# microsoft/Sora

Hardware: AMD Instinct MI355X
Metric: IQ Msamples/s through 802.11a 54 Mbps RX PHY (higher is better)
Workload: dtype int16 IQ / u8 path metrics

## Files before the change

### sora_amd/csrc/dev_vit16.h

```cpp
#pragma once
#include <hip/hip_runtime.h>
#include "kernels.h"
#include "dev_viterbi.h"

namespace sora {
namespace {

template <int WIN, int LOOK> struct Geom16 {
    static constexpr int kMaxWalk = (WIN + LOOK + 7) / 8 + 2;
    static constexpr int P = kMaxWalk;
    static constexpr int kPathBytes = 40;
};

template <int WIN, int LOOK> struct Lds16 {
    uint16_t ring[Geom16<WIN, LOOK>::P][4][64];
    union {
        uint32_t udump[4][64];
        uint16_t ops[4][24][2];
        uint16_t ops2[2][4][24][2];
    };
    uint32_t path[8][Geom16<WIN, LOOK>::kPathBytes / 4];
};

constexpr unsigned kW[4] = { 0u, 21u, 42u, 63u };

__device__ __forceinline__ unsigned v_of_lane(unsigned l)
{
    const unsigned b0 = l & 1u, b1 = (l >> 1) & 1u, b2 = (l >> 2) & 1u, b3 = (l >> 3) & 1u;
    const unsigned c3 = b2, c1 = b3, c0 = b0 ^ c3, c2 = b1 ^ c3;
    return c0 | (c1 << 1) | (c2 << 2) | (c3 << 3);
}
__device__ __forceinline__ unsigned lane_of_v(unsigned v)
{
    const unsigned c0 = v & 1u, c1 = (v >> 1) & 1u, c2 = (v >> 2) & 1u, c3 = (v >> 3) & 1u;
    return c0 ^ (c2 << 1) ^ (c1 << 3) ^ (c3 ? 7u : 0u);
}
__device__ __forceinline__ unsigned rev6u(unsigned x) { return __brev(x) >> 26; }

template <int CTRL> __device__ __forceinline__ unsigned dppx(unsigned v) { return (unsigned)__builtin_amdgcn_update_dpp(0, (int)v, CTRL, 0xF, 0xF, true); }

__device__ __forceinline__ unsigned partner(unsigned v, int ph)
{
    switch (ph) {
    case 0: return dppx<0x140>(v);
    case 1: return dppx<0x1B>(v);
    case 2: return dppx<0x141>(v);
    case 3: return dppx<0x4E>(v);
    case 4: return dppx<0x128>(v);
    default: return dppx<0xB1>(v);
    }
}

struct Vit16 {
    unsigned U[4];
    unsigned MX[24];
    unsigned MY[6];
    unsigned sadr[3][4];
};

template <int WHICH, int P>
__device__ __forceinline__ void acs16(Vit16& V, int t24, unsigned a, unsigned b, unsigned pos512[3])
{
    const int ph = t24 % 6, k = t24 % 8;
    const unsigned Kp = (WHICH == 0 ? 14u : 7u) * kFld + (kOne << k);
    unsigned bm;
    if (WHICH == 0)      bm = (a ^ V.MX[t24]) + (b ^ V.MY[ph]);
    else if (WHICH == 1) bm = a ^ V.MX[t24];
    else                 bm = b ^ V.MX[t24];
    const unsigned bo = Kp - bm;
    const int rx = ph == 0 ? 2 : ph == 1 ? 1 : 0;
    unsigned N[4];
#pragma unroll
    for (int i = 0; i < 4; i++) {
        const unsigned X = V.U[i], Y = partner(V.U[i ^ rx], ph);
        const bool wb = (kW[i] >> (5 - ph)) & 1u;
        N[i] = wb ? pk_min16(X + bo, Y + bm) : pk_min16(X + bm, Y + bo);
    }
#pragma unroll
    for (int i = 0; i < 4; i++) V.U[i] = N[i];
    if (k == 7) {
        const int jb = t24 / 8;
#pragma unroll
        for (int i = 0; i < 4; i++) {
            const unsigned w = bank_word(V.U[i]);
            const unsigned addr = V.sadr[jb][i] + pos512[jb];
            asm volatile("ds_write_b16 %0, %1" : : "v"(addr), "v"(w) : "memory");
            V.U[i] &= 0xFE00FE00u;
        }
    }
}

__device__ __forceinline__ unsigned row_min_u32(unsigned v)
{
    v = min(v, dppx<0xB1>(v)); v = min(v, dppx<0x4E>(v)); v = min(v, dppx<0x141>(v)); v = min(v, dppx<0x128>(v));
    return v;
}
__device__ __forceinline__ unsigned row_pkmin(unsigned v)
{
    v = pk_min16(v, dppx<0xB1>(v)); v = pk_min16(v, dppx<0x4E>(v)); v = pk_min16(v, dppx<0x141>(v)); v = pk_min16(v, dppx<0x128>(v));
    return v;
}
__device__ __forceinline__ unsigned wave_min_u32(unsigned v) { return (unsigned)__builtin_amdgcn_readfirstlane((int)dpp_min_u32_wave(v)); }
__device__ __forceinline__ unsigned wave_max_u32(unsigned v) { return ~wave_min_u32(~v); }

template <int CR, int WIN, int LOOK, int BITS>
struct Forward16 {
    static constexpr int P = Geom16<WIN, LOOK>::P, GB = Puncture<CR>::GB, GS = Puncture<CR>::GS, CW = Puncture<CR>::CW;
    static constexpr int NV = Puncture<CR>::NV;
    struct Chunk { uint32_t v[CW]; };
    struct Raw { SoftRaw r[NV]; };

    Vit16 V;
    unsigned row, half;
    uint32_t my_j;
    SoftCursor<BITS, CW> cur[NV];
    uint32_t my_base;
    const uint8_t* soft;
    uint16_t* my_ops;
    const uint4* row_ops;
    uint32_t pos;
    unsigned pos512[3];
    uint32_t tr, nsteps;
    uint32_t next_thr;
    bool all_done;

    __device__ __forceinline__ void init(Lds16<WIN, LOOK>& S, const uint8_t* __restrict__ soft_, uint32_t my_soft_off, uint32_t my_first, uint32_t my_last, unsigned start,
                                         uint32_t nsteps_)
    {
        const unsigned lane = threadIdx.x & 63, l16 = lane & 15;
        row = lane >> 4; half = lane & 1u;
        const unsigned v0 = v_of_lane(l16);
        nsteps = nsteps_;
#pragma unroll
        for (int i = 0; i < 4; i++) V.U[i] = (v0 ^ kW[i]) == 0 ? 0u : start;
        const unsigned ring_base = (unsigned)(uintptr_t)&S.ring[0][0][0];
#pragma unroll
        for (int jb = 0; jb < 3; jb++)
#pragma unroll
            for (int i = 0; i < 4; i++) V.sadr[jb][i] = ring_base + ((row * 64u + rev6u(rol6(v0 ^ kW[i], jb == 0 ? 2 : jb == 1 ? 4 : 0))) << 1);
#pragma unroll
        for (int t = 0; t < 24; t++) {
            const int ph = t % 6, k = t % 8;
            const unsigned n = rol6(v0, ph + 1);
            const bool vb = (v0 >> (5 - ph)) & 1u;
            const unsigned ma = (__popc(n & 0155) & 1) ? 7u * kFld : 0u, mb = (__popc(n & 0117) & 1) ? 7u * kFld : 0u;
            const unsigned mx = Puncture<CR>::which_of(ph) == 2 ? mb : ma;
            V.MX[t] = vb ? ((mx ^ (7u * kFld)) | (kOne << k)) : mx;
            if (t < 6) V.MY[t] = vb ? (mb ^ (7u * kFld)) : mb;
        }
        tr = 0; pos = 0;
        my_j = l16 >> 1;
#pragma unroll
        for (int v = 0; v < NV; v++) cur[v].init(my_soft_off, my_first + my_j + 8u * v, my_last);
        my_base = my_soft_off + my_first + my_j;
        soft = soft_;
        my_ops = &S.ops[row][my_j][half];
        row_ops = reinterpret_cast<const uint4*>(&S.ops[row][0][0]);
        set_row_pos();
        clear_ops(S);
    }
    __device__ __forceinline__ bool going() const { return tr < nsteps && !all_done; }

    __device__ __forceinline__ void normalize()
    {
        const unsigned m = row_pkmin(pk_min16(pk_min16(V.U[0], V.U[1]), pk_min16(V.U[2], V.U[3])));
#pragma unroll
        for (int i = 0; i < 4; i++) V.U[i] -= m;
    }
    static __device__ __forceinline__ uint32_t pos_of(uint32_t p, int jb) { const uint32_t q = p + 512u * (uint32_t)jb; return min(q, q - 512u * (uint32_t)P); }
    __device__ __forceinline__ void set_row_pos()
    {
        pos512[0] = pos; pos512[1] = pos_of(pos, 1); pos512[2] = pos_of(pos512[1], 1);
    }
    __device__ __forceinline__ void end_row() { pos = pos_of(pos512[2], 1); set_row_pos(); }
    __device__ __forceinline__ Raw fetch(uint32_t c) const
    {
        Raw R;
#pragma unroll
        for (int v = 0; v < NV; v++) R.r[v] = cur[v].fetch(soft, c);
        return R;
    }
    __device__ __forceinline__ void put(const Raw& R, uint16_t* mine) const
    {
#pragma unroll
        for (int v = 0; v < NV; v++) soft_put(mine + 16 * v, cur[v], R.r[v]);
    }
    __device__ __forceinline__ void clear_ops(Lds16<WIN, LOOK>& S) const
    {
        if constexpr (BITS == kSoftScaled) {
            static_assert(sizeof(S.ops2) == 3 * 64 * 4, "three dwords per lane");
            uint32_t* z = reinterpret_cast<uint32_t*>(&S.ops2[0][0][0][0]) + (threadIdx.x & 63);
            z[0] = 0u; z[64] = 0u; z[128] = 0u;
            lds_fence();
        }
    }
    __device__ __forceinline__ uint32_t fast_base(uint32_t c0) const { return my_base + c0 * (uint32_t)CW; }
    template <int DC> __device__ __forceinline__ Raw fetch_at(uint32_t p) const
    {
        static_assert(BITS == kSoftScaled, "one byte per value");
        Raw R;
#pragma unroll
        for (int v = 0; v < NV; v++) { R.r[v].sh = 0; R.r[v].w = soft[(size_t)p + (size_t)(DC * CW + 8 * v)]; }
        return R;
    }
    static __device__ __forceinline__ Chunk get(const uint4* table)
    {
        Chunk K;
#pragma unroll
        for (int i = 0; i < (CW + 3) / 4; i++) {
            const uint4 x = table[i];
            K.v[4 * i] = x.x; K.v[4 * i + 1] = x.y;
            if (4 * i + 2 < CW) { K.v[4 * i + 2] = x.z; K.v[4 * i + 3] = x.w; }
        }
        return K;
    }
    __device__ __forceinline__ Chunk unpack(const Raw& R) const
    {
        put(R, my_ops);
        lds_fence();
        const Chunk K = get(row_ops);
        lds_fence();
        return K;
    }
    __device__ __forceinline__ void group(const Chunk& K, int h, int i0)
    {
        const int k0 = i0 / GS * GB, t24 = 12 * h + i0;
        acs16<0, P>(V, t24, K.v[k0], K.v[k0 + 1], pos512);
        if (CR != 0) acs16<1, P>(V, t24 + 1, K.v[k0 + 2], 0, pos512);
        if (CR == 2) acs16<2, P>(V, t24 + 2, 0, K.v[k0 + 3], pos512);
        if ((t24 + GS) % 8 == 0) normalize();
    }
    __device__ __forceinline__ void fast_chunk(const Chunk& K, int h)
    {
#pragma unroll
        for (int g = 0; g < 12 / GS; g++) group(K, h, g * GS);
        tr += 12;
    }
    template <typename CHECK> __device__ __forceinline__ void slow_chunk(const Chunk& K, int h, CHECK& check)
    {
#pragma unroll
        for (int g = 0; g < 12 / GS; g++) {
            if (going()) {
                group(K, h, g * GS);
                tr += GS;
                check(12 * h + g * GS + GS - 1);
            }
        }
    }
    template <typename CHECK> __device__ __forceinline__ void chunk(const Chunk& K, int h, CHECK& check)
    {
        if (tr + 12 <= nsteps && next_thr > tr + 12) fast_chunk(K, h); else slow_chunk(K, h, check);
    }
};

template <int WIN, int LOOK, bool LANE_OB = false>
__device__ __noinline__ void trace16(unsigned lds_off, unsigned U0, unsigned U1, unsigned U2, unsigned U3, uint32_t tr_, uint32_t ob_, uint32_t pj_, uint32_t k_,
                                     uint32_t my_cnt, uint8_t* my_out)
{
    using G = Geom16<WIN, LOOK>;
    constexpr int P = G::P, K = G::kMaxWalk;
    constexpr int NR = K - 1, NF = NR / 4, NW = K / 4 + 1;
    static_assert(NR % 4 == 0 || NR % 4 == 2, "the walk's words are packed in pairs");
    static_assert(NW * 4 <= G::kPathBytes && NW >= WIN / 32 + 1, "the stream's registers hold a window and fit Lds16::path");
    typedef __attribute__((address_space(3))) Lds16<WIN, LOOK> lds_t;
    typedef __attribute__((address_space(3))) const uint16_t lds_u16;
    lds_t& S = *(lds_t*)(uintptr_t)lds_off;
    auto uni = [](uint32_t v) { return (uint32_t)__builtin_amdgcn_readfirstlane((int)v); };
    const uint32_t tr = uni(tr_), ob = LANE_OB ? ob_ : uni(ob_), pj = uni(pj_), k = uni(k_);
    const unsigned lane = threadIdx.x & 63, row = lane >> 4, l16 = lane & 15, half = lane & 1u;
    const unsigned v0 = v_of_lane(l16);
    const unsigned U[4] = { U0, U1, U2, U3 };
    const uint32_t j = (tr - 1) >> 3, nn = tr - 8u * j, m_lo = ob >> 3;
    const unsigned rowbase = (unsigned)(uintptr_t)&S.ring[0][row][0], sh = 8u * half;
    auto ring_j = [&](unsigned idx) -> unsigned { return *(lds_u16*)(uintptr_t)(rowbase + pj + (idx << 1)); };
#pragma unroll
    for (int i = 0; i < 4; i++) S.udump[i][lane] = U[i];
    lds_fence();
    unsigned key[2] = { 0xFFFFFFFFu, 0xFFFFFFFFu };
#pragma unroll
    for (int i = 0; i < 4; i++) {
        const unsigned st = rol6(v0 ^ kW[i], tr);
        unsigned lastA, lastB;
        if (k == 7) { const unsigned w = ring_j(rev6u(st)); lastA = (w >> 7) & 1u; lastB = (w >> 15) & 1u; }
        else { lastA = (U[i] >> k) & 1u; lastB = (U[i] >> (17 + k)) & 1u; }
        const unsigned mA = ((U[i] & 0xFFFFu) >> 9 << 1) | lastA, mB = (U[i] >> 25 << 1) | lastB;
        key[0] = min(key[0], (mA << 8) | (st << 2)); key[1] = min(key[1], (mB << 8) | (st << 2));
    }
    const unsigned kA = row_min_u32(key[0]), kB = row_min_u32(key[1]);
    const unsigned st = ((half ? kB : kA) >> 2) & 0x3Fu;
    const unsigned s0 = rol6(st, 6u - tr % 6u);
    const unsigned b4 = (s0 >> 4) & 1u, b5 = (s0 >> 5) & 1u;
    const unsigned ri = b4 | (b5 << 1);
    const unsigned sl = lane_of_v((s0 ^ (b4 ? 21u : 0u) ^ (b5 ? 42u : 0u)) & 15u);
    const unsigned Ust = S.udump[ri][row * 16u + sl];
    unsigned H;
    if (nn == 8) H = (ring_j(rev6u(st)) >> sh) & 0xFFu;
    else H = ((Ust >> (17u * half)) & 0xFFu) & ((1u << nn) - 1u);
    unsigned q = rev6u(((st >> nn) | rev6u(H & 0x3Fu)) & 0x3Fu);
    unsigned pr[NR / 2];
    uint32_t p = pj;
#pragma unroll
    for (int i = 1; i < K; i++) {
        uint32_t d;
        p = __builtin_sub_overflow(p, 512u, &d) ? 512u * (uint32_t)(P - 1) : d;
        unsigned base = rowbase + p;
        asm volatile("" : "+v"(base));
        const unsigned raw = *(lds_u16*)(uintptr_t)(base + (q << 1));
        q = __builtin_amdgcn_ubfe(raw, sh, 6u);
        const int s = K - 1 - i;
        if (s & 1) pr[s >> 1] = raw << 16; else pr[s >> 1] |= raw;
    }
    unsigned R[NW];
    const unsigned sel = 0x06040200u + 0x01010101u * half;
#pragma unroll
    for (int w = 0; w < NF; w++) R[w] = __builtin_amdgcn_perm(pr[2 * w + 1], pr[2 * w], sel);
    if (NR % 4 == 0) R[NF] = H;
    else R[NF] = __builtin_amdgcn_perm(H, pr[2 * NF], 0x0C040200u + 0x00000101u * half);
    const uint32_t sfirst = (uint32_t)(K - 1) - (j - m_lo);
    bool fast = !LANE_OB;
    if (!LANE_OB) {
        const bool whole = my_cnt == (uint32_t)WIN && sfirst == 1u && (((uintptr_t)my_out + m_lo) & 3u) == 0;
        fast = __ballot(!(whole || my_cnt == 0)) == 0;
    }
    if (fast) {
        if (my_cnt != 0 && l16 < 2) {
            uint32_t* o = reinterpret_cast<uint32_t*>(my_out + m_lo);
#pragma unroll
            for (int dw = 0; dw < WIN / 32; dw++) o[dw] = __builtin_amdgcn_alignbit(R[dw + 1], R[dw], 14);
        }
    } else {
        __attribute__((address_space(3))) uint32_t* pw = S.path[row * 2u + half];
        if (l16 < 2) {
#pragma unroll
            for (int w = 0; w < NW; w++) pw[w] = R[w];
        }
        lds_fence();
        __attribute__((address_space(3))) const uint8_t* pth = (__attribute__((address_space(3))) const uint8_t*)pw;
        const uint32_t nbytes = my_cnt >> 3;
        for (uint32_t z = l16 >> 1; z < nbytes; z += 8) {
            const uint32_t sb = sfirst + z;
            my_out[m_lo + z] = (uint8_t)(((unsigned)pth[sb] >> 6) | (((unsigned)pth[sb + 1] & 0x3Fu) << 2));
        }
    }
    lds_fence();
}

}
}
```

### sora_amd/csrc/k_vit16.hip

```cpp
#include <hip/hip_runtime.h>

#include "dev_vit16.h"

namespace sora {

namespace {

template <int CR, int WIN, int LOOK, int BITS>
__device__ __forceinline__ void forward16(Lds16<WIN, LOOK>& S, const uint8_t* __restrict__ soft, uint32_t my_soft_off, uint32_t my_nsoft,
                                          uint32_t nstepsA, uint32_t nstepsB, uint32_t my_tr_end, bool my_valid, uint8_t* my_out)
{
    using F16 = Forward16<CR, WIN, LOOK, BITS>;
    using Chunk = typename F16::Chunk;
    using Raw = typename F16::Raw;
    constexpr int GS = F16::GS;
    F16 F;
    F.init(S, soft, my_soft_off, 0, max(my_nsoft, 1u) - 1u, 0x18u * kFld, wave_max_u32(max(nstepsA, nstepsB)));

    uint32_t ob = 0;
    bool my_done = !my_valid;

    auto trace = [&](uint32_t my_cnt, int t24_last) {
        trace16<WIN, LOOK>((unsigned)(uintptr_t)&S, F.V.U[0], F.V.U[1], F.V.U[2], F.V.U[3], F.tr, ob, F16::pos_of(F.pos, t24_last / 8), (uint32_t)(t24_last % 8), my_cnt, my_out);
    };
    auto next_event = [&]() -> uint32_t {
        const uint32_t mine = my_done ? kNever : my_tr_end;
        return min(ob + (uint32_t)(WIN + LOOK + 6), wave_min_u32(mine));
    };
    F.next_thr = next_event();
    F.all_done = wave_min_u32(my_done ? 1u : 0u) != 0u;
    auto check = [&](int t24_last) {
        if (F.tr >= F.next_thr) {
            const bool partial = F.tr >= ob + (uint32_t)(WIN + LOOK + 6);
            uint32_t cnt = 0;
            if (!my_done) {
                if (F.tr >= my_tr_end) { cnt = my_tr_end - ob - 6; my_done = true; }
                else if (partial) cnt = WIN;
            }
            if (wave_max_u32(cnt) != 0u) { trace(cnt, t24_last); F.clear_ops(S); }
            if (partial) ob += WIN;
            F.next_thr = next_event();
            F.all_done = wave_min_u32(my_done ? 1u : 0u) != 0u;
        }
    };

    uint16_t* my_ops2[2] = { &S.ops2[0][F.row][F.my_j][F.half], &S.ops2[1][F.row][F.my_j][F.half] };
    const uint4* row_ops2[2] = { reinterpret_cast<const uint4*>(&S.ops2[0][F.row][0][0]), reinterpret_cast<const uint4*>(&S.ops2[1][F.row][0][0]) };
    auto stage = [&](const Raw& R, int t) { F.put(R, my_ops2[t]); };
    auto collect = [&](int t) -> Chunk { lds_fence(); return F16::get(row_ops2[t]); };
    auto fast_chunk_mid = [&](const Chunk& K, int h, Chunk& Knext, int tnext) {
#pragma unroll
        for (int g = 0; g < 12 / GS; g++) {
            if (g == (12 / GS) / 2) Knext = collect(tnext);
            F.group(K, h, g * GS);
        }
        F.tr += 12;
    };

    uint32_t c = 0;
    Raw b0 = F.fetch(0), b1 = F.fetch(1), b2, b3;
    while (F.going()) {
        const uint32_t lim = min(F.nsteps, F.next_thr - 1);
        uint32_t rows = lim > F.tr ? (lim - F.tr) / 24 : 0;
        if (rows >= 2) {
            Chunk Ka, Kb;
            b2 = F.fetch(c + 2);
            stage(b0, 0); Ka = collect(0); lds_fence();
            if constexpr (BITS == kSoftScaled) {
                uint32_t p = F.fast_base(c);
                for (; rows >= 2; rows -= 2) {
                    b3 = F.template fetch_at<3>(p); stage(b1, 1); fast_chunk_mid(Ka, 0, Kb, 1);
                    b0 = F.template fetch_at<4>(p); stage(b2, 0); fast_chunk_mid(Kb, 1, Ka, 0);
                    F.end_row();
                    b1 = F.template fetch_at<5>(p); stage(b3, 1); fast_chunk_mid(Ka, 0, Kb, 1);
                    b2 = F.template fetch_at<6>(p); stage(b0, 0); fast_chunk_mid(Kb, 1, Ka, 0);
                    F.end_row();
                    c += 4; p += 4u * (uint32_t)F16::CW;
                }
            } else {
                for (; rows >= 2; rows -= 2) {
                    b3 = F.fetch(c + 3); stage(b1, 1); fast_chunk_mid(Ka, 0, Kb, 1);
                    b0 = F.fetch(c + 4); stage(b2, 0); fast_chunk_mid(Kb, 1, Ka, 0);
                    F.end_row();
                    b1 = F.fetch(c + 5); stage(b3, 1); fast_chunk_mid(Ka, 0, Kb, 1);
                    b2 = F.fetch(c + 6); stage(b0, 0); fast_chunk_mid(Kb, 1, Ka, 0);
                    F.end_row();
                    c += 4;
                }
            }
            lds_fence();
        }
        if (!(F.tr < F.nsteps)) break;
        b2 = F.fetch(c + 2);
        if (rows) F.fast_chunk(F.unpack(b0), 0); else F.chunk(F.unpack(b0), 0, check);
        if (!F.going()) break;
        b3 = F.fetch(c + 3);
        if (rows) F.fast_chunk(F.unpack(b1), 1); else F.chunk(F.unpack(b1), 1, check);
        F.end_row();
        b0 = b2; b1 = b3;
        c += 2;
    }
}

template <int WIN, int LOOK, int BITS>
__device__ __forceinline__ void viterbi16_body(const VitJob* __restrict__ jobs, const uint32_t* __restrict__ njobs3, uint32_t njobs_single, uint32_t stride,
                                               const uint8_t* __restrict__ soft, uint8_t* __restrict__ out)
{
    __shared__ Lds16<WIN, LOOK> S;
    uint32_t n[3] = { njobs_single, 0, 0 };
    if (njobs3) { n[0] = njobs3[0]; n[1] = njobs3[1]; n[2] = njobs3[2]; }
    uint32_t w = uni(blockIdx.x), list = 0;
    while (list < 3 && w >= (n[list] + 7) / 8) { w -= (n[list] + 7) / 8; list++; }
    if (list >= 3) return;
    const uint32_t njobs = uni(n[list]);
    jobs += (size_t)list * stride;
    const unsigned lane = threadIdx.x & 63, row = lane >> 4, half = lane & 1u;
    const uint32_t fa = 8u * w + 2u * row, fb = fa + 1u;
    const bool hasA = fa < njobs, hasB = fb < njobs;
    const VitJob& GA = jobs[hasA ? fa : 8u * w];
    const VitJob& GBj = jobs[hasB ? fb : (hasA ? fa : 8u * w)];
    const uint32_t code_rate = uni(jobs[8u * w].code_rate);
    const uint32_t gsd = code_rate == 0 ? 2u : code_rate == 2 ? 4u : 3u, gss = code_rate == 0 ? 1u : code_rate == 2 ? 3u : 2u;
    const uint32_t nstepsA = hasA ? GA.nsoft / gsd * gss : 0u, nstepsB = hasB ? GBj.nsoft / gsd * gss : 0u;
    const VitJob& Mine = half ? GBj : GA;
    const bool my_valid = half ? hasB : hasA;
    const uint32_t my_tr_end = Mine.length * 8u + 16u + 6u;
    uint8_t* my_out = out + Mine.out_off;
    if (code_rate == 0)      forward16<0, WIN, LOOK, BITS>(S, soft, Mine.soft_off, Mine.nsoft, nstepsA, nstepsB, my_tr_end, my_valid, my_out);
    else if (code_rate == 1) forward16<1, WIN, LOOK, BITS>(S, soft, Mine.soft_off, Mine.nsoft, nstepsA, nstepsB, my_tr_end, my_valid, my_out);
    else                     forward16<2, WIN, LOOK, BITS>(S, soft, Mine.soft_off, Mine.nsoft, nstepsA, nstepsB, my_tr_end, my_valid, my_out);
}

}

__global__ void __launch_bounds__(64) k_viterbi16(const VitJob* __restrict__ jobs, const uint32_t* __restrict__ njobs3, uint32_t njobs_single, uint32_t stride,
        const uint8_t* __restrict__ soft, uint8_t* __restrict__ out)
{ viterbi16_body<256, 24, kSoftScaled>(jobs, njobs3, njobs_single, stride, soft, out); }
__global__ void __launch_bounds__(64) k_viterbi16_p3(const VitJob* __restrict__ jobs, const uint32_t* __restrict__ njobs3, uint32_t njobs_single, uint32_t stride,
        const uint8_t* __restrict__ soft, uint8_t* __restrict__ out)
{ viterbi16_body<256, 24, 3>(jobs, njobs3, njobs_single, stride, soft, out); }
__global__ void __launch_bounds__(64) k_viterbi16_11n(const VitJob* __restrict__ jobs, const uint32_t* __restrict__ njobs3, uint32_t njobs_single,
        uint32_t stride, const uint8_t* __restrict__ soft, uint8_t* __restrict__ out)
{ viterbi16_body<192, 36, 8>(jobs, njobs3, njobs_single, stride, soft, out); }

}
```

Baseline: 55870.

## Overlap Viterbi traceback walk with forward ACS steps in 16-bit decoder

When a full window is ready and conditions allow, the traceback is started but its per-step LDS walk is interleaved with the next two rows of forward ACS groups via a hook, instead of running as a separate serial trace. Survivor bank writes that would overwrite ring entries still needed by the walk are held in registers and flushed once the walk finishes. This aims to hide traceback latency behind forward compute, at the cost of more registers, more code paths and a fallback when alignment or window conditions fail.

```diff
diff --git a/sora_amd/csrc/dev_vit16.h b/sora_amd/csrc/dev_vit16.h
--- a/sora_amd/csrc/dev_vit16.h
+++ b/sora_amd/csrc/dev_vit16.h
@@ -87,6 +87,46 @@
             asm volatile("ds_write_b16 %0, %1" : : "v"(addr), "v"(w) : "memory");
             V.U[i] &= 0xFE00FE00u;
         }
+    }
+}
+
+struct BankStore16 {
+    __device__ __forceinline__ void operator()(const Vit16& V, const unsigned pos512[3], int jb, const unsigned w[4]) const
+    {
+#pragma unroll
+        for (int i = 0; i < 4; i++) {
+            const unsigned addr = V.sadr[jb][i] + pos512[jb];
+            asm volatile("ds_write_b16 %0, %1" : : "v"(addr), "v"(w[i]) : "memory");
+        }
+    }
+};
+
+template <int WHICH, int P, typename BANK>
+__device__ __forceinline__ void acs16(Vit16& V, int t24, unsigned a, unsigned b, unsigned pos512[3], BANK&& bank)
+{
+    const int ph = t24 % 6, k = t24 % 8;
+    const unsigned Kp = (WHICH == 0 ? 14u : 7u) * kFld + (kOne << k);
+    unsigned bm;
+    if (WHICH == 0)      bm = (a ^ V.MX[t24]) + (b ^ V.MY[ph]);
+    else if (WHICH == 1) bm = a ^ V.MX[t24];
+    else                 bm = b ^ V.MX[t24];
+    const unsigned bo = Kp - bm;
+    const int rx = ph == 0 ? 2 : ph == 1 ? 1 : 0;
+    unsigned N[4];
+#pragma unroll
+    for (int i = 0; i < 4; i++) {
+        const unsigned X = V.U[i], Y = partner(V.U[i ^ rx], ph);
+        const bool wb = (kW[i] >> (5 - ph)) & 1u;
+        N[i] = wb ? pk_min16(X + bo, Y + bm) : pk_min16(X + bm, Y + bo);
+    }
+#pragma unroll
+    for (int i = 0; i < 4; i++) V.U[i] = N[i];
+    if (k == 7) {
+        const int jb = t24 / 8;
+        unsigned w[4];
+#pragma unroll
+        for (int i = 0; i < 4; i++) { w[i] = bank_word(V.U[i]); V.U[i] &= 0xFE00FE00u; }
+        bank(V, pos512, jb, w);
     }
 }
 
@@ -250,6 +290,37 @@
     template <typename CHECK> __device__ __forceinline__ void chunk(const Chunk& K, int h, CHECK& check)
     {
         if (tr + 12 <= nsteps && next_thr > tr + 12) fast_chunk(K, h); else slow_chunk(K, h, check);
+    }
+    struct NoHook { __device__ __forceinline__ void operator()(int) const {} };
+    template <typename HOOK, typename BANK> __device__ __forceinline__ void group(const Chunk& K, int h, int i0, HOOK&& hook, BANK&& bank)
+    {
+        const int k0 = i0 / GS * GB, t24 = 12 * h + i0;
+        hook(t24);
+        acs16<0, P>(V, t24, K.v[k0], K.v[k0 + 1], pos512, bank);
+        if (CR != 0) { hook(t24 + 1); acs16<1, P>(V, t24 + 1, K.v[k0 + 2], 0, pos512, bank); }
+        if (CR == 2) { hook(t24 + 2); acs16<2, P>(V, t24 + 2, 0, K.v[k0 + 3], pos512, bank); }
+        if ((t24 + GS) % 8 == 0) normalize();
+    }
+    template <typename BANK> __device__ __forceinline__ void fast_chunk(const Chunk& K, int h, BANK&& bank)
+    {
+#pragma unroll
+        for (int g = 0; g < 12 / GS; g++) group(K, h, g * GS, NoHook{}, bank);
+        tr += 12;
+    }
+    template <typename CHECK, typename BANK> __device__ __forceinline__ void slow_chunk(const Chunk& K, int h, CHECK& check, BANK&& bank)
+    {
+#pragma unroll
+        for (int g = 0; g < 12 / GS; g++) {
+            if (going()) {
+                group(K, h, g * GS, NoHook{}, bank);
+                tr += GS;
+                check(12 * h + g * GS + GS - 1);
+            }
+        }
+    }
+    template <typename CHECK, typename BANK> __device__ __forceinline__ void chunk(const Chunk& K, int h, CHECK& check, BANK&& bank)
+    {
+        if (tr + 12 <= nsteps && next_thr > tr + 12) fast_chunk(K, h, bank); else slow_chunk(K, h, check, bank);
     }
 };
 
@@ -345,5 +416,106 @@
     lds_fence();
 }
 
-}
-}
+template <int WIN, int LOOK>
+__device__ __forceinline__ void trace16_start(unsigned lds_off, const unsigned U[4], uint32_t tr, uint32_t pj, uint32_t k, unsigned& H_, unsigned& q_)
+{
+    typedef __attribute__((address_space(3))) Lds16<WIN, LOOK> lds_t;
+    typedef __attribute__((address_space(3))) const uint16_t lds_u16;
+    lds_t& S = *(lds_t*)(uintptr_t)lds_off;
+    const unsigned lane = threadIdx.x & 63, row = lane >> 4, l16 = lane & 15, half = lane & 1u;
+    const unsigned v0 = v_of_lane(l16);
+    const uint32_t j = (tr - 1) >> 3, nn = tr - 8u * j;
+    const unsigned rowbase = (unsigned)(uintptr_t)&S.ring[0][row][0], sh = 8u * half;
+    auto ring_j = [&](unsigned idx) -> unsigned { return *(lds_u16*)(uintptr_t)(rowbase + pj + (idx << 1)); };
+#pragma unroll
+    for (int i = 0; i < 4; i++) S.udump[i][lane] = U[i];
+    lds_fence();
+    unsigned key[2] = { 0xFFFFFFFFu, 0xFFFFFFFFu };
+#pragma unroll
+    for (int i = 0; i < 4; i++) {
+        const unsigned st = rol6(v0 ^ kW[i], tr);
+        unsigned lastA, lastB;
+        if (k == 7) { const unsigned w = ring_j(rev6u(st)); lastA = (w >> 7) & 1u; lastB = (w >> 15) & 1u; }
+        else { lastA = (U[i] >> k) & 1u; lastB = (U[i] >> (17 + k)) & 1u; }
+        const unsigned mA = ((U[i] & 0xFFFFu) >> 9 << 1) | lastA, mB = (U[i] >> 25 << 1) | lastB;
+        key[0] = min(key[0], (mA << 8) | (st << 2)); key[1] = min(key[1], (mB << 8) | (st << 2));
+    }
+    const unsigned kA = row_min_u32(key[0]), kB = row_min_u32(key[1]);
+    const unsigned st = ((half ? kB : kA) >> 2) & 0x3Fu;
+    const unsigned s0 = rol6(st, 6u - tr % 6u);
+    const unsigned b4 = (s0 >> 4) & 1u, b5 = (s0 >> 5) & 1u;
+    const unsigned ri = b4 | (b5 << 1);
+    const unsigned sl = lane_of_v((s0 ^ (b4 ? 21u : 0u) ^ (b5 ? 42u : 0u)) & 15u);
+    const unsigned Ust = S.udump[ri][row * 16u + sl];
+    unsigned H;
+    if (nn == 8) H = (ring_j(rev6u(st)) >> sh) & 0xFFu;
+    else H = ((Ust >> (17u * half)) & 0xFFu) & ((1u << nn) - 1u);
+    unsigned q = rev6u(((st >> nn) | rev6u(H & 0x3Fu)) & 0x3Fu);
+    H_ = H; q_ = q;
+}
+
+template <int WIN, int LOOK>
+__device__ __forceinline__ void path16_words(const unsigned* pr, unsigned H, unsigned half, unsigned* R)
+{
+    constexpr int NR = Geom16<WIN, LOOK>::kMaxWalk - 1, NF = NR / 4;
+    const unsigned sel = 0x06040200u + 0x01010101u * half;
+#pragma unroll
+    for (int w = 0; w < NF; w++) R[w] = __builtin_amdgcn_perm(pr[2 * w + 1], pr[2 * w], sel);
+    if (NR % 4 == 0) R[NF] = H;
+    else R[NF] = __builtin_amdgcn_perm(H, pr[2 * NF], 0x0C040200u + 0x00000101u * half);
+}
+
+template <int WIN, int LOOK>
+__device__ __noinline__ unsigned trace16_begin(unsigned lds_off, unsigned U0, unsigned U1, unsigned U2, unsigned U3, uint32_t tr_, uint32_t pj_, uint32_t k_)
+{
+    auto uni = [](uint32_t v) { return (uint32_t)__builtin_amdgcn_readfirstlane((int)v); };
+    const unsigned U[4] = { U0, U1, U2, U3 };
+    unsigned H, q;
+    trace16_start<WIN, LOOK>(lds_off, U, uni(tr_), uni(pj_), uni(k_), H, q);
+    lds_fence();
+    return (H << 8) | q;
+}
+
+template <int WIN, int LOOK>
+struct Walk16 {
+    using G = Geom16<WIN, LOOK>;
+    static constexpr int P = G::P, K = G::kMaxWalk, NR = K - 1, NW = K / 4 + 1;
+    typedef __attribute__((address_space(3))) const uint16_t lds_u16;
+    unsigned q, H, raw, rowbase, half;
+    uint32_t p;
+    unsigned pr[NR / 2];
+
+    __device__ __forceinline__ void begin(Lds16<WIN, LOOK>& S, unsigned started, uint32_t pj)
+    {
+        const unsigned lane = threadIdx.x & 63;
+        half = lane & 1u;
+        rowbase = (unsigned)(uintptr_t)&S.ring[0][lane >> 4][0];
+        q = started & 0xFFu; H = started >> 8; p = pj;
+    }
+    __device__ __forceinline__ void issue()
+    {
+        uint32_t d;
+        p = __builtin_sub_overflow(p, 512u, &d) ? 512u * (uint32_t)(P - 1) : d;
+        unsigned base = rowbase + p;
+        asm volatile("" : "+v"(base));
+        raw = *(lds_u16*)(uintptr_t)(base + (q << 1));
+    }
+    __device__ __forceinline__ void take(int i)
+    {
+        q = __builtin_amdgcn_ubfe(raw, 8u * half, 6u);
+        const int s = K - 1 - i;
+        if (s & 1) pr[s >> 1] = raw << 16; else pr[s >> 1] |= raw;
+    }
+    __device__ __forceinline__ void emit(uint32_t* o, bool mine) const
+    {
+        unsigned R[NW];
+        path16_words<WIN, LOOK>(pr, H, half, R);
+        if (mine) {
+#pragma unroll
+            for (int dw = 0; dw < WIN / 32; dw++) o[dw] = __builtin_amdgcn_alignbit(R[dw + 1], R[dw], 14);
+        }
+    }
+};
+
+}
+}
diff --git a/sora_amd/csrc/k_vit16.hip b/sora_amd/csrc/k_vit16.hip
--- a/sora_amd/csrc/k_vit16.hip
+++ b/sora_amd/csrc/k_vit16.hip
@@ -1,4 +1,6 @@
 #include <hip/hip_runtime.h>
+
+#include <type_traits>
 
 #include "dev_vit16.h"
 
@@ -29,9 +31,42 @@
     };
     F.next_thr = next_event();
     F.all_done = wave_min_u32(my_done ? 1u : 0u) != 0u;
+
+    using W16 = Walk16<WIN, LOOK>;
+    constexpr int kHeld = W16::NR / 8;
+    W16 W;
+    bool hold = false, w_mine = false;
+    uint32_t w_mlo = 0;
+    unsigned D[3][4], dpos[3] = { 0, 0, 0 }, D2[kHeld][4], d2pos[kHeld];
+    auto bank_or_hold = [&](const Vit16& V, const unsigned pos512[3], int jb, const unsigned w[4]) {
+#pragma unroll
+        for (int i = 0; i < 4; i++) D[jb][i] = w[i];
+        dpos[jb] = pos512[jb];
+        if (!hold) BankStore16{}(V, pos512, jb, w);
+    };
+    auto store_word = [&](unsigned addr, unsigned w) { asm volatile("ds_write_b16 %0, %1" : : "v"(addr), "v"(w) : "memory"); };
+    auto may_overlap = [&](int t24_last, uint32_t ends) -> bool {
+        const uint32_t m_lo = ob >> 3, j = (F.tr - 1) >> 3;
+        const uint32_t boundary = F.tr + (uint32_t)(23 - t24_last);
+        const uint32_t lim = min(F.nsteps, min(ob + (uint32_t)(2 * WIN + LOOK + 6), ends) - 1u);
+        if (!(F.tr < ends && boundary + 48u <= lim && (uint32_t)(W16::K - 1) - (j - m_lo) == 1u)) return false;
+        return __ballot(!my_done && (((uintptr_t)my_out + m_lo) & 3u) != 0) == 0;
+    };
     auto check = [&](int t24_last) {
         if (F.tr >= F.next_thr) {
             const bool partial = F.tr >= ob + (uint32_t)(WIN + LOOK + 6);
+            if (partial) {
+                const uint32_t ends = wave_min_u32(my_done ? kNever : my_tr_end);
+                if (may_overlap(t24_last, ends)) {
+                    const uint32_t pj = F16::pos_of(F.pos, t24_last / 8);
+                    W.begin(S, trace16_begin<WIN, LOOK>((unsigned)(uintptr_t)&S, F.V.U[0], F.V.U[1], F.V.U[2], F.V.U[3], F.tr, pj, (uint32_t)(t24_last % 8)), pj);
+                    F.clear_ops(S);
+                    hold = true; w_mine = !my_done && (threadIdx.x & 15) < 2; w_mlo = ob >> 3;
+                    ob += WIN;
+                    F.next_thr = min(ob + (uint32_t)(WIN + LOOK + 6), ends);
+                    return;
+                }
+            }
             uint32_t cnt = 0;
             if (!my_done) {
                 if (F.tr >= my_tr_end) { cnt = my_tr_end - ob - 6; my_done = true; }
@@ -48,13 +83,28 @@
     const uint4* row_ops2[2] = { reinterpret_cast<const uint4*>(&S.ops2[0][F.row][0][0]), reinterpret_cast<const uint4*>(&S.ops2[1][F.row][0][0]) };
     auto stage = [&](const Raw& R, int t) { F.put(R, my_ops2[t]); };
     auto collect = [&](int t) -> Chunk { lds_fence(); return F16::get(row_ops2[t]); };
-    auto fast_chunk_mid = [&](const Chunk& K, int h, Chunk& Knext, int tnext) {
+    auto fast_chunk_mid = [&](const Chunk& K, int h, Chunk& Knext, int tnext, auto&& hook, auto&& bank) {
 #pragma unroll
         for (int g = 0; g < 12 / GS; g++) {
             if (g == (12 / GS) / 2) Knext = collect(tnext);
-            F.group(K, h, g * GS);
+            F.group(K, h, g * GS, hook, bank);
         }
         F.tr += 12;
+    };
+    auto walk_step = [&](int n) {
+        if (n >= 1 && n <= W16::NR) W.take(n);
+        if (n < W16::NR) W.issue();
+        if (n == W16::NR) {
+#pragma unroll
+            for (int jb = 0; jb < 3; jb++)
+#pragma unroll
+                for (int i = 0; i < 4; i++) store_word(F.V.sadr[jb][i] + dpos[jb], D[jb][i]);
+#pragma unroll
+            for (int b = 0; b < kHeld; b++)
+#pragma unroll
+                for (int i = 0; i < 4; i++) store_word(F.V.sadr[b % 3][i] + d2pos[b], D2[b][i]);
+        }
+        if (n == W16::NR + 1) W.emit(reinterpret_cast<uint32_t*>(my_out + w_mlo), w_mine);
     };
 
     uint32_t c = 0;
@@ -66,36 +116,43 @@
             Chunk Ka, Kb;
             b2 = F.fetch(c + 2);
             stage(b0, 0); Ka = collect(0); lds_fence();
-            if constexpr (BITS == kSoftScaled) {
-                uint32_t p = F.fast_base(c);
-                for (; rows >= 2; rows -= 2) {
-                    b3 = F.template fetch_at<3>(p); stage(b1, 1); fast_chunk_mid(Ka, 0, Kb, 1);
-                    b0 = F.template fetch_at<4>(p); stage(b2, 0); fast_chunk_mid(Kb, 1, Ka, 0);
-                    F.end_row();
-                    b1 = F.template fetch_at<5>(p); stage(b3, 1); fast_chunk_mid(Ka, 0, Kb, 1);
-                    b2 = F.template fetch_at<6>(p); stage(b0, 0); fast_chunk_mid(Kb, 1, Ka, 0);
-                    F.end_row();
-                    c += 4; p += 4u * (uint32_t)F16::CW;
-                }
-            } else {
-                for (; rows >= 2; rows -= 2) {
-                    b3 = F.fetch(c + 3); stage(b1, 1); fast_chunk_mid(Ka, 0, Kb, 1);
-                    b0 = F.fetch(c + 4); stage(b2, 0); fast_chunk_mid(Kb, 1, Ka, 0);
-                    F.end_row();
-                    b1 = F.fetch(c + 5); stage(b3, 1); fast_chunk_mid(Ka, 0, Kb, 1);
-                    b2 = F.fetch(c + 6); stage(b0, 0); fast_chunk_mid(Kb, 1, Ka, 0);
-                    F.end_row();
-                    c += 4;
-                }
-            }
+            uint32_t p = BITS == kSoftScaled ? F.fast_base(c) : 0u;
+            auto turn = [&](auto walking) {
+                constexpr bool kWalk = decltype(walking)::value;
+                auto fx = [&](auto dc) -> Raw {
+                    if constexpr (BITS == kSoftScaled) return F.template fetch_at<decltype(dc)::value>(p); else return F.fetch(c + (uint32_t)decltype(dc)::value);
+                };
+                auto hook = [&](int r) {
+                    if constexpr (kWalk) return [&, r](int t24) { walk_step(24 * r + t24); }; else return typename F16::NoHook{};
+                };
+                auto bank = [&](int r) {
+                    if constexpr (kWalk) return [&, r](const Vit16& V, const unsigned pos512[3], int jb, const unsigned w[4]) {
+                        const int b = 3 * r + jb;
+                        if (b < kHeld) {
+#pragma unroll
+                            for (int i = 0; i < 4; i++) D2[b][i] = w[i];
+                            d2pos[b] = pos512[jb];
+                        } else BankStore16{}(V, pos512, jb, w);
+                    }; else return BankStore16{};
+                };
+                b3 = fx(std::integral_constant<int, 3>{}); stage(b1, 1); fast_chunk_mid(Ka, 0, Kb, 1, hook(0), bank(0));
+                b0 = fx(std::integral_constant<int, 4>{}); stage(b2, 0); fast_chunk_mid(Kb, 1, Ka, 0, hook(0), bank(0));
+                F.end_row();
+                b1 = fx(std::integral_constant<int, 5>{}); stage(b3, 1); fast_chunk_mid(Ka, 0, Kb, 1, hook(1), bank(1));
+                b2 = fx(std::integral_constant<int, 6>{}); stage(b0, 0); fast_chunk_mid(Kb, 1, Ka, 0, hook(1), bank(1));
+                F.end_row();
+                c += 4; p += 4u * (uint32_t)F16::CW; rows -= 2;
+            };
+            if (hold) { turn(std::true_type{}); hold = false; }
+            while (rows >= 2) turn(std::false_type{});
             lds_fence();
         }
         if (!(F.tr < F.nsteps)) break;
         b2 = F.fetch(c + 2);
-        if (rows) F.fast_chunk(F.unpack(b0), 0); else F.chunk(F.unpack(b0), 0, check);
+        if (rows) F.fast_chunk(F.unpack(b0), 0, bank_or_hold); else F.chunk(F.unpack(b0), 0, check, bank_or_hold);
         if (!F.going()) break;
         b3 = F.fetch(c + 3);
-        if (rows) F.fast_chunk(F.unpack(b1), 1); else F.chunk(F.unpack(b1), 1, check);
+        if (rows) F.fast_chunk(F.unpack(b1), 1, bank_or_hold); else F.chunk(F.unpack(b1), 1, check, bank_or_hold);
         F.end_row();
         b0 = b2; b1 = b3;
         c += 2;
```

Measured after the change: 54210. 3.0% lower.
